# huettern/edison

Measured on AMD Instinct MI355X. Metric: MFCC frames/sec + KWS inferences/sec (whole node) at 1/2/4/8 MI355X, higher is better.
Workload: dtype f32

## Files before the change

### edison_amd/csrc/tables.c

```c
#include <math.h>
#include <stdio.h>
#include <stdlib.h>
#include <string.h>

#include "../../include/edison_hip.h"
#include "edison_internal.h"

#define MEL_HIGH_FREQUENCY_Q 1127.0
#define MEL_BREAK_FREQUENCY_HERTZ 700.0

static double hz2mel(double hz) { return MEL_HIGH_FREQUENCY_Q * log(1.0 + hz / MEL_BREAK_FREQUENCY_HERTZ); }

static void linspace(double a, double b, int n, double *out)
{
	double step = n > 1 ? (b - a) / (double)(n - 1) : 0.0;
	for (int i = 0; i < n; i++) out[i] = (double)i * step + a;
	if (n > 1) out[n - 1] = b;
}

int ed_gen_mel_weight_matrix(int num_mel_bins, int num_spectrogram_bins, double sample_rate,
                             double lower_edge_hertz, double upper_edge_hertz, double *W)
{
	if (num_mel_bins < 1 || num_spectrogram_bins < 2 || W == NULL) return EDISON_E_ARGUMENT;
	double *lin = (double *)malloc(sizeof(double) * (size_t)num_spectrogram_bins);
	double *edge = (double *)malloc(sizeof(double) * (size_t)(num_mel_bins + 2));
	if (!lin || !edge) { free(lin); free(edge); return EDISON_E_NO_MEMORY; }
	linspace(0.0, sample_rate / 2.0, num_spectrogram_bins, lin);
	linspace(hz2mel(lower_edge_hertz), hz2mel(upper_edge_hertz), num_mel_bins + 2, edge);
	memset(W, 0, sizeof(double) * (size_t)num_mel_bins);
	for (int k = 1; k < num_spectrogram_bins; k++)
	{
		double m = hz2mel(lin[k]);
		double *row = W + (size_t)k * num_mel_bins;
		for (int j = 0; j < num_mel_bins; j++)
		{
			double up = (m - edge[j]) / (edge[j + 1] - edge[j]);
			double dn = (edge[j + 2] - m) / (edge[j + 2] - edge[j + 1]);
			double w = up < dn ? up : dn;
			row[j] = w > 0.0 ? w : 0.0;
		}
	}
	free(lin); free(edge);
	return EDISON_OK;
}

static const unsigned char g_b128_group[4][16] = {
	{0, 1, 2, 3, 12, 13, 14, 15, 20, 21, 22, 23, 24, 25, 26, 27},
	{4, 5, 6, 7, 8, 9, 10, 11, 16, 17, 18, 19, 28, 29, 30, 31},
	{32, 33, 34, 35, 44, 45, 46, 47, 52, 53, 54, 55, 56, 57, 58, 59},
	{36, 37, 38, 39, 40, 41, 42, 43, 48, 49, 50, 51, 60, 61, 62, 63}};

static int mel_read_passes(int first4[2][EDISON_NUM_MEL][4], int NLO, int NHI, const int *col_band, const int *half)
{
	int total = 0;
	for (int part = 0; part < 2; part++)
		for (int t = 0; t < (part == 0 ? NLO : NHI); t++)
			for (int second = 0; second < 2; second++)
				for (int g = 0; g < 4; g++)
				{
					int n_in_slot[16] = {0}, held[16][16], worst = 1;
					for (int i = 0; i < 16; i++)
					{
						const int l = g_b128_group[g][i], b = col_band[l & 15];
						const int q = first4[part][part == 0 ? b : 31 - b][l >> 4] + t;
						const int addr = 2 * q + (second ? 1 - half[l] : half[l]), slot = addr & 15;
						int k = 0;
						while (k < n_in_slot[slot] && held[slot][k] != addr) k++;
						if (k == n_in_slot[slot]) held[slot][n_in_slot[slot]++] = addr;
						if (n_in_slot[slot] > worst) worst = n_in_slot[slot];
					}
					total += worst;
				}
	return total;
}

static void choose_lane_assignment(int first4[2][EDISON_NUM_MEL][4], int NLO, int NHI, int *col_band, int *half)
{
	int best = -1, cb[16], hf[64];
	uint32_t rng = 12345u;
	for (int start = 0; start < 8; start++)
	{
		for (int c = 0; c < 16; c++) cb[c] = c;
		for (int l = 0; l < 64; l++) hf[l] = l & 1;
		if (start > 0)
		{
			for (int c = 15; c > 0; c--)
			{
				rng = rng * 1664525u + 1013904223u;
				const int k = (int)((rng >> 8) % (uint32_t)(c + 1)), tmp = cb[c];
				cb[c] = cb[k]; cb[k] = tmp;
			}
			for (int l = 0; l < 64; l++) { rng = rng * 1664525u + 1013904223u; hf[l] = (int)((rng >> 16) & 1u); }
		}
		int cost = mel_read_passes(first4, NLO, NHI, cb, hf), improved = 1;
		while (improved)
		{
			improved = 0;
			for (int l = 0; l < 64; l++)
			{
				hf[l] ^= 1;
				const int c2 = mel_read_passes(first4, NLO, NHI, cb, hf);
				if (c2 < cost) { cost = c2; improved = 1; } else hf[l] ^= 1;
			}
			for (int a = 0; a < 16; a++)
				for (int b = a + 1; b < 16; b++)
				{
					int tmp = cb[a]; cb[a] = cb[b]; cb[b] = tmp;
					const int c2 = mel_read_passes(first4, NLO, NHI, cb, hf);
					if (c2 < cost) { cost = c2; improved = 1; } else { tmp = cb[a]; cb[a] = cb[b]; cb[b] = tmp; }
				}
		}
		if (best < 0 || cost < best)
		{
			best = cost;
			memcpy(col_band, cb, sizeof(cb));
			memcpy(half, hf, sizeof(hf));
		}
	}
}

int ed_build_mfcc_tables(int variant, double sample_rate, double lower_edge_hertz, double upper_edge_hertz,
                         double mel_mtx_scale, ed_mfcc_tables_t *out, char *err, size_t err_cap)
{
	const int NMEL = EDISON_NUM_MEL;
	const int nbins = (variant == EDISON_MFCC_A) ? EDISON_FRAME_LEN / 2 : EDISON_FRAME_LEN / 2 + 1;
	if (variant != EDISON_MFCC_A && variant != EDISON_MFCC_B && variant != EDISON_MFCC_TF) return EDISON_E_ARGUMENT;
	memset(out, 0, sizeof(*out));
	const double spec_scale = (variant == EDISON_MFCC_B) ? 0.5 / 1024.0 / sqrt(2.0) : 0.5;

	for (int l = 0; l < 64; l++)
		for (int p = 0; p < 8; p++)
		{
			double a = -2.0 * M_PI * (double)(l * p) / 512.0;
			out->tw1[p][l][0] = (float)cos(a); out->tw1[p][l][1] = (float)sin(a);
			a = -2.0 * M_PI * (double)((l & 7) * p) / 64.0;
			out->tw2[p][l][0] = (float)cos(a); out->tw2[p][l][1] = (float)sin(a);
		}
	for (int m = 0; m < 4; m++)
		for (int l = 0; l < 64; l++)
		{
			const int k0 = ED_K0(l);
			double a = -2.0 * M_PI * (double)(k0 + 64 * m) / 1024.0;
			out->twp[m][l][0] = (float)cos(a); out->twp[m][l][1] = (float)sin(a);
		}

	double *W = (double *)malloc(sizeof(double) * (size_t)nbins * NMEL);
	if (!W) return EDISON_E_NO_MEMORY;
	int r = ed_gen_mel_weight_matrix(NMEL, nbins, sample_rate, lower_edge_hertz, upper_edge_hertz, W);
	if (r != EDISON_OK) { free(W); return r; }
	(void)mel_mtx_scale;
	int q0[EDISON_NUM_MEL], nq[EDISON_NUM_MEL], ks[EDISON_NUM_MEL], ke[EDISON_NUM_MEL];
	for (int j = 0; j < NMEL; j++)
	{
		int first = -1, last = -1;
		for (int k = 0; k < nbins; k++)
			if (W[(size_t)k * NMEL + j] != 0.0) { if (first < 0) first = k; last = k; }
		if (first < 0) { first = 0; last = -1; }
		ks[j] = first; ke[j] = last + 1;
		q0[j] = first / 4;
		nq[j] = last >= first ? last / 4 - first / 4 + 1 : 0;
	}
	int NLO = 1, NHI = 1;
	for (int b = 0; b < 16; b++)
	{
		if ((nq[b] + 3) / 4 > NLO) NLO = (nq[b] + 3) / 4;
		if ((nq[31 - b] + 3) / 4 > NHI) NHI = (nq[31 - b] + 3) / 4;
	}
	if (NLO > ED_MEL_NLO_MAX || NHI > ED_MEL_NHI_MAX)
	{
		if (err) snprintf(err, err_cap, "mel filterbank needs %d+%d spectrum quads per lane, the kernel's budget is %d+%d",
		                  NLO, NHI, ED_MEL_NLO_MAX, ED_MEL_NHI_MAX);
		free(W);
		return EDISON_E_NO_IMPL;
	}
	const char *force_wide = getenv("EDISON_FORCE_WIDE_MEL");
	if (NLO <= 2 && NHI <= 5 && !(force_wide && force_wide[0] == '1')) { NLO = 2; NHI = 5; }
	else { NLO = ED_MEL_NLO_MAX; NHI = ED_MEL_NHI_MAX; }
	out->mel_NLO = NLO; out->mel_NHI = NHI;
	int first4[2][EDISON_NUM_MEL][4];
	for (int j = 0; j < NMEL; j++)
		for (int rr = 0; rr < 4; rr++)
			for (int part = 0; part < 2; part++)
			{
				const int N = part == 0 ? NLO : NHI;
				int s4 = q0[j] + rr * ((nq[j] + 3) / 4);
				if (s4 > ED_SPEC_QUADS - N) s4 = ED_SPEC_QUADS - N;
				if (s4 < 0) s4 = 0;
				first4[part][j][rr] = s4;
			}
	int col_band[16], half[64];
	choose_lane_assignment(first4, NLO, NHI, col_band, half);
	for (int l = 0; l < 64; l++)
	{
		const int b = col_band[l & 15], rr = l >> 4;
		out->mel_band[l] = b;
		out->mel_half[l] = half[l];
		for (int part = 0; part < 2; part++)
		{
			const int j = part == 0 ? b : 31 - b, N = part == 0 ? NLO : NHI;
			const int per = (nq[j] + 3) / 4;
			const int pq0 = q0[j] + rr * per;
			int pq1 = pq0 + per;
			if (pq1 > q0[j] + nq[j]) pq1 = q0[j] + nq[j];
			const int s4 = first4[part][j][rr];
			if (part == 0) out->mel_slo4[l] = s4; else out->mel_shi4[l] = s4;
			for (int t = 0; t < N; t++)
				for (int c = 0; c < 4; c++)
				{
					const int q = s4 + t, k = 4 * q + c;
					const int mine = q >= pq0 && q < pq1 && k >= ks[j] && k < ke[j] && k < nbins;
					out->mel_w4[(part == 0 ? 0 : NLO) + t][l][c] = mine ? (float)(spec_scale * W[(size_t)k * NMEL + j]) : 0.0f;
				}
		}
	}
	free(W);

	double dscale = (variant == EDISON_MFCC_B) ? 1.0 / 64.0 : 1.0 / sqrt(2.0 * (double)NMEL);
	for (int l = 0; l < 64; l++)
	{
		int c = l & 31, h = l >> 5;
		for (int n = 0; n < 8; n++)
		{
			int nn = n + 8 * h;
			out->dct4[n / 4][l][n % 4] =
			    (float)(dscale * 2.0 * cos(M_PI * (double)c * (double)(2 * nn + 1) / (double)(2 * NMEL)));
		}
	}
	out->spec_scale = (float)spec_scale;
	out->log_offset = 1e-6f;
	out->always_log = (variant == EDISON_MFCC_B) ? 0 : 1;
	if (variant == EDISON_MFCC_TF)
	{
		out->has_window = 1;
		for (int n = 0; n < EDISON_FRAME_LEN; n++)
			out->window2[n / 2][n % 2] = (float)(0.5 - 0.5 * cos(2.0 * M_PI * (double)n / (double)EDISON_FRAME_LEN));
	}
	return EDISON_OK;
}

enum { LDS_R128, LDS_W128, LDS_W64, LDS_W32, LDS_R2_64, LDS_RTN32 };

static void lds_passes(int kind, const int *addr, int *free_passes, int *extra_passes)
{
	const int n_groups = kind == LDS_R128 ? 4 : kind == LDS_W128 ? 8 : kind == LDS_W64 || kind == LDS_R2_64 ? 4 : 2;
	const int n_banks = kind == LDS_R128 ? 64 : 32;
	const int n_dwords = kind == LDS_R128 || kind == LDS_W128 ? 4 : kind == LDS_W64 || kind == LDS_R2_64 ? 2 : 1;
	const int per = 64 / n_groups;
	*free_passes = 0; *extra_passes = 0;
	for (int g = 0; g < n_groups; g++)
	{
		int n_in_bank[64] = {0}, held[64][32], worst = 0;
		for (int i = 0; i < per; i++)
		{
			const int l = kind == LDS_R128 ? g_b128_group[g][i] : g * per + i;
			if (addr[l] < 0) continue;
			for (int d = 0; d < n_dwords; d++)
			{
				const int dw = addr[l] / 4 + d, bank = dw % n_banks;
				int k = 0;
				while (k < n_in_bank[bank] && held[bank][k] != dw) k++;
				if (k == n_in_bank[bank]) held[bank][n_in_bank[bank]++] = dw;
				if (n_in_bank[bank] > worst) worst = n_in_bank[bank];
			}
		}
		if (worst > 0) { *free_passes += 1; *extra_passes += worst - 1; }
	}
}

int ed_mfcc2_lds_account(const ed_mfcc_tables_t *tab, int t2_stride, int wave, ed_lds_row_t *rows, int max_rows)
{
	if (!tab || !rows || max_rows < ED_LDS_ROWS_MAX || wave < 0 || t2_stride < 64) return EDISON_E_ARGUMENT;
	const int NLO = tab->mel_NLO, NHI = tab->mel_NHI;
	const int melw = 4 * ED2_TABLE_FLOATS;
	const int xbuf = 4 * (ED2_TABLE_FLOATS + (NLO + NHI) * 256 + wave * ED2_XBUF_FLOATS);
	const int S2 = xbuf + 4 * ED2_S_OFF, Lb2 = xbuf + 4 * ED2_L_OFF;
	int n = 0, addr[64], f, e;
#define ROW(nm, k) { rows[n].name = nm; rows[n].kind = k; rows[n].instructions = 0; rows[n].free_passes = 0; rows[n].extra_passes = 0; n++; }
#define ADD() { lds_passes(rows[n - 1].kind, addr, &f, &e); rows[n - 1].free_passes += f; rows[n - 1].extra_passes += e; }
#define ADD1() { ADD(); rows[n - 1].instructions++; }
	ROW("queue draw: ds_add_rtn_u32, lane 0", LDS_RTN32);
	for (int l = 0; l < 64; l++) addr[l] = l == 0 ? xbuf + 4 * (12 - wave) * ED2_XBUF_FLOATS : -1;
	ADD1();
	ROW("transpose 2 stores: ds_write_b128 xc4[stride (lane & 7) + (lane >> 3) + 8 q]", LDS_W128);
	for (int q = 0; q < 8; q++)
	{
		for (int l = 0; l < 64; l++) addr[l] = xbuf + 16 * (t2_stride * (l & 7) + (l >> 3) + 8 * q);
		ADD1();
	}
	ROW("transpose 2 reads: ds_read_b128 xc4[stride c + lane]", LDS_R128);
	for (int c = 0; c < 8; c++)
	{
		for (int l = 0; l < 64; l++) addr[l] = xbuf + 16 * (t2_stride * c + l);
		ADD1();
	}
	ROW("split twiddles: ds_read2st64_b64 tpl[64 m + lane], two m each", LDS_R2_64);
	for (int m = 0; m < 4; m++)
	{
		for (int l = 0; l < 64; l++) addr[l] = 4 * 512 + 8 * (64 * m + l);
		ADD();
		rows[n - 1].instructions = (m + 2) / 2;
	}
	ROW("spectrum stores: ds_write_b64 S2[k0 + 64 m]", LDS_W64);
	for (int m = 0; m < 4; m++)
	{
		for (int l = 0; l < 64; l++) addr[l] = S2 + 8 * (ED_K0(l) + 64 * m);
		ADD1();
	}
	ROW("spectrum stores, mirrored: ds_write_b64 S2[512 - k0 - 64 m]", LDS_W64);
	for (int m = 0; m < 4; m++)
	{
		for (int l = 0; l < 64; l++) addr[l] = S2 + 8 * (512 - ED_K0(l) - 64 * m);
		ADD1();
	}
	ROW("spectrum store S2[256]: ds_write_b64, lane 0", LDS_W64);
	for (int l = 0; l < 64; l++) addr[l] = l == 0 ? S2 + 8 * 256 : -1;
	ADD1();
	ROW("mel spectrum reads: ds_read_b128 S4[2 (first + t) + half], S4[2 (first + t) + 1 - half]", LDS_R128);
	for (int part = 0; part < 2; part++)
		for (int t = 0; t < (part == 0 ? NLO : NHI); t++)
			for (int second = 0; second < 2; second++)
			{
				for (int l = 0; l < 64; l++)
				{
					const int first = part == 0 ? tab->mel_slo4[l] : tab->mel_shi4[l], h = tab->mel_half[l];
					addr[l] = S2 + 16 * (2 * (first + t) + (second ? 1 - h : h));
					if (addr[l] + 16 > S2 + 8 * 516) return EDISON_E_ARGUMENT;
				}
				ADD1();
			}
	ROW("mel weight reads: ds_read_b128 melw4[64 t + lane]", LDS_R128);
	for (int t = 0; t < NLO + NHI; t++)
	{
		for (int l = 0; l < 64; l++) addr[l] = melw + 16 * (64 * t + l);
		ADD1();
	}
	ROW("DCT input store: ds_write_b32 Lb2[l_idx]", LDS_W32);
	for (int l = 0; l < 64; l++) addr[l] = Lb2 + 4 * (2 * (16 * ((l >> 4) & 1) + tab->mel_band[l]) + (l >> 5));
	ADD1();
	ROW("DCT input reads: ds_read_b128 L4[0..3], L4 = Lb2 + 16 (lane & 1) + 8 (lane >> 5)", LDS_R128);
	for (int i = 0; i < 4; i++)
	{
		for (int l = 0; l < 64; l++) addr[l] = Lb2 + 8 * (16 * (l & 1) + 8 * (l >> 5)) + 16 * i;
		ADD1();
	}
	ROW("DCT table reads: ds_read_b128 dctl[lane], dctl[64 + lane]", LDS_R128);
	for (int i = 0; i < 2; i++)
	{
		for (int l = 0; l < 64; l++) addr[l] = 16 * (64 * i + l);
		ADD1();
	}
#undef ROW
#undef ADD
#undef ADD1
	return n;
}

int ed_build_exact_tables(double sample_rate, double lower_edge_hertz, double upper_edge_hertz, double mel_mtx_scale, ed_exact_tables_t *out)
{
	const int NMEL = EDISON_NUM_MEL, nbins = EDISON_FRAME_LEN / 2 + 1;
	memset(out, 0, sizeof(*out));
	for (int k = 0; k < 512; k++)
	{
		out->tw[k][0] = cos(-2.0 * M_PI * (double)k / 1024.0);
		out->tw[k][1] = sin(-2.0 * M_PI * (double)k / 1024.0);
	}
	for (int c = 0; c < NMEL; c++)
		for (int n = 0; n < NMEL; n++)
			out->dct[c][n] = 2.0 * cos(M_PI * (double)c * (double)(2 * n + 1) / (double)(2 * NMEL));
	double *W = (double *)malloc(sizeof(double) * (size_t)nbins * NMEL);
	if (!W) return EDISON_E_NO_MEMORY;
	int r = ed_gen_mel_weight_matrix(NMEL, nbins, sample_rate, lower_edge_hertz, upper_edge_hertz, W);
	if (r != EDISON_OK) { free(W); return r; }
	int off = 0;
	for (int j = 0; j < NMEL; j++)
	{
		int first = -1, last = -1;
		for (int k = 0; k < nbins; k++)
			if (W[(size_t)k * NMEL + j] != 0.0) { if (first < 0) first = k; last = k; }
		const int len = first < 0 ? 0 : last - first + 1;
		if (off + len > ED_EXACT_TAPS_MAX) { free(W); return EDISON_E_NO_IMPL; }
		out->mel_off[j] = off; out->mel_k0[j] = first < 0 ? 0 : first; out->mel_len[j] = len;
		for (int t = 0; t < len; t++) out->mel_w[off + t] = mel_mtx_scale * W[(size_t)(first + t) * NMEL + j];
		off += len;
	}
	out->mel_div = mel_mtx_scale;
	free(W);
	return EDISON_OK;
}
```

Measured before the change: 1.507 billion.

## Search mel lane assignment with slack-aware start offsets to cut LDS bank conflicts

Adds a host-side randomized local search over the mel filterbank lane assignment. It varies band-to-column mapping, per-lane start quads within the range where the weights are nonzero, and the half-swap bit, scoring each candidate with an LDS bank-conflict model. The goal is fewer extra passes on the ds_read_b128 spectrum reads in the MFCC kernel. Table build time goes up, which a memo mitigates, and the model of bank behavior may not match the hardware.

Result: no change. 1.519 billion (median of 5 runs) (+0.8%).

```diff
diff --git a/edison_amd/csrc/tables.c b/edison_amd/csrc/tables.c
--- a/edison_amd/csrc/tables.c
+++ b/edison_amd/csrc/tables.c
@@ -1,4 +1,6 @@
+#include <limits.h>
 #include <math.h>
+#include <pthread.h>
 #include <stdio.h>
 #include <stdlib.h>
 #include <string.h>
@@ -44,11 +46,63 @@
 	return EDISON_OK;
 }
 
+enum { LDS_R128, LDS_W128, LDS_W64, LDS_W32, LDS_R2_64, LDS_RTN32 };
+
 static const unsigned char g_b128_group[4][16] = {
 	{0, 1, 2, 3, 12, 13, 14, 15, 20, 21, 22, 23, 24, 25, 26, 27},
 	{4, 5, 6, 7, 8, 9, 10, 11, 16, 17, 18, 19, 28, 29, 30, 31},
 	{32, 33, 34, 35, 44, 45, 46, 47, 52, 53, 54, 55, 56, 57, 58, 59},
 	{36, 37, 38, 39, 40, 41, 42, 43, 48, 49, 50, 51, 60, 61, 62, 63}};
+
+static int lds_groups(int kind) { return kind == LDS_R128 ? 4 : kind == LDS_W128 ? 8 : kind == LDS_W64 || kind == LDS_R2_64 ? 4 : 2; }
+
+static int lds_group_passes(int kind, int g, const int *addr, int *crowding)
+{
+	const int n_banks = kind == LDS_R128 ? 64 : 32;
+	const int n_dwords = kind == LDS_R128 || kind == LDS_W128 ? 4 : kind == LDS_W64 || kind == LDS_R2_64 ? 2 : 1;
+	const int per = 64 / lds_groups(kind);
+	int n_in_bank[64] = {0}, held[64][32], worst = 0, step = 1;
+	if (n_dwords == 4)
+	{
+		step = 4;
+		for (int i = 0; i < per; i++)
+		{
+			const int l = kind == LDS_R128 ? g_b128_group[g][i] : g * per + i;
+			if (addr[l] >= 0 && addr[l] % 16 != 0) step = 1;
+		}
+	}
+	for (int i = 0; i < per; i++)
+	{
+		const int l = kind == LDS_R128 ? g_b128_group[g][i] : g * per + i;
+		if (addr[l] < 0) continue;
+		for (int d = 0; d < n_dwords; d += step)
+		{
+			const int dw = addr[l] / 4 + d, bank = dw % n_banks;
+			int k = 0;
+			while (k < n_in_bank[bank] && held[bank][k] != dw) k++;
+			if (k == n_in_bank[bank]) held[bank][n_in_bank[bank]++] = dw;
+			if (n_in_bank[bank] > worst) worst = n_in_bank[bank];
+		}
+	}
+	if (crowding)
+	{
+		*crowding = 0;
+		for (int bank = 0; bank < n_banks; bank += step) *crowding += step * n_in_bank[bank] * n_in_bank[bank];
+	}
+	return worst;
+}
+
+static void lds_passes(int kind, const int *addr, int *free_passes, int *extra_passes)
+{
+	*free_passes = 0; *extra_passes = 0;
+	for (int g = 0; g < lds_groups(kind); g++)
+	{
+		const int worst = lds_group_passes(kind, g, addr, NULL);
+		if (worst > 0) { *free_passes += 1; *extra_passes += worst - 1; }
+	}
+}
+
+static int mel_read_slot(int first, int t, int second, int half) { return 2 * (first + t) + (second ? 1 - half : half); }
 
 static int mel_read_passes(int first4[2][EDISON_NUM_MEL][4], int NLO, int NHI, const int *col_band, const int *half)
 {
@@ -119,6 +173,144 @@
 	}
 }
 
+typedef struct
+{
+	int first_lo[2][16][4], first_hi[2][16][4], half_free[16][4];
+} mel_freedom_t;
+
+typedef struct
+{
+	int col_band[16], first[2][16][4], half[16][4];
+} mel_assignment_t;
+
+static long mel_group_cost(const mel_assignment_t *a, int part, int N, int g)
+{
+	long cost = 0;
+	int addr[64];
+	for (int t = 0; t < N; t++)
+		for (int second = 0; second < 2; second++)
+		{
+			int crowding;
+			for (int i = 0; i < 16; i++)
+			{
+				const int l = g_b128_group[g][i], b = a->col_band[l & 15], rr = l >> 4;
+				addr[l] = 16 * mel_read_slot(a->first[part][b][rr], t, second, a->half[b][rr]);
+			}
+			cost += (1L << 20) * lds_group_passes(LDS_R128, g, addr, &crowding) + crowding;
+		}
+	return cost;
+}
+
+static long mel_cost(const mel_assignment_t *a, int NLO, int NHI, long limit)
+{
+	long cost = 0;
+	for (int g = 0; g < 4 && cost < limit; g++)
+	{
+		cost += mel_group_cost(a, 0, NLO, g);
+		if (cost < limit) cost += mel_group_cost(a, 1, NHI, g);
+	}
+	return cost;
+}
+
+static void refine_lane_assignment(const mel_freedom_t *fr, int NLO, int NHI, mel_assignment_t *a)
+{
+	const int N[2] = {NLO, NHI};
+	int group_of[64];
+	for (int g = 0; g < 4; g++)
+		for (int i = 0; i < 16; i++) group_of[g_b128_group[g][i]] = g;
+	for (int round = 0, improved = 1; improved && round < 64; round++)
+	{
+		improved = 0;
+		for (int c = 0; c < 16; c++)
+			for (int rr = 0; rr < 4; rr++)
+			{
+				const int b = a->col_band[c], g = group_of[c + 16 * rr];
+				for (int part = 0; part < 2; part++)
+				{
+					int best_first = a->first[part][b][rr];
+					long best = mel_group_cost(a, part, N[part], g);
+					for (int s = fr->first_lo[part][b][rr]; s <= fr->first_hi[part][b][rr]; s++)
+					{
+						a->first[part][b][rr] = s;
+						const long c2 = mel_group_cost(a, part, N[part], g);
+						if (c2 < best) { best = c2; best_first = s; improved = 1; }
+					}
+					a->first[part][b][rr] = best_first;
+				}
+				if (fr->half_free[b][rr])
+				{
+					const long c1 = mel_group_cost(a, 0, NLO, g) + mel_group_cost(a, 1, NHI, g);
+					a->half[b][rr] ^= 1;
+					if (mel_group_cost(a, 0, NLO, g) + mel_group_cost(a, 1, NHI, g) < c1) improved = 1; else a->half[b][rr] ^= 1;
+				}
+			}
+		long cost = mel_cost(a, NLO, NHI, LONG_MAX);
+		for (int x = 0; x < 16; x++)
+			for (int y = x + 1; y < 16; y++)
+			{
+				if (group_of[x] == group_of[y]) continue;
+				int tmp = a->col_band[x]; a->col_band[x] = a->col_band[y]; a->col_band[y] = tmp;
+				const long c2 = mel_cost(a, NLO, NHI, cost);
+				if (c2 < cost) { cost = c2; improved = 1; } else { tmp = a->col_band[x]; a->col_band[x] = a->col_band[y]; a->col_band[y] = tmp; }
+			}
+	}
+}
+
+#ifndef ED_MEL_SEARCH_STARTS
+#define ED_MEL_SEARCH_STARTS 24
+#endif
+#define ED_MEL_SEARCH_MEMO 8
+static void search_lane_assignment(const mel_freedom_t *fr, int NLO, int NHI, mel_assignment_t *a)
+{
+	static struct { int used, NLO, NHI; mel_freedom_t fr; mel_assignment_t given, found; } memo[ED_MEL_SEARCH_MEMO];
+	static int memo_next = 0;
+	static pthread_mutex_t memo_lock = PTHREAD_MUTEX_INITIALIZER;
+	const mel_assignment_t given = *a;
+	pthread_mutex_lock(&memo_lock);
+	for (int i = 0; i < ED_MEL_SEARCH_MEMO; i++)
+		if (memo[i].used && memo[i].NLO == NLO && memo[i].NHI == NHI && !memcmp(&memo[i].fr, fr, sizeof(*fr)) && !memcmp(&memo[i].given, &given, sizeof(given)))
+		{
+			*a = memo[i].found;
+			pthread_mutex_unlock(&memo_lock);
+			return;
+		}
+	pthread_mutex_unlock(&memo_lock);
+	long best = -1;
+	uint32_t rng = 12345u;
+	for (int start = 0; start < ED_MEL_SEARCH_STARTS; start++)
+	{
+		mel_assignment_t c = given;
+		if (start > 0)
+		{
+			for (int x = 15; x > 0; x--)
+			{
+				rng = rng * 1664525u + 1013904223u;
+				const int k = (int)((rng >> 8) % (uint32_t)(x + 1)), tmp = c.col_band[x];
+				c.col_band[x] = c.col_band[k]; c.col_band[k] = tmp;
+			}
+			for (int b = 0; b < 16; b++)
+				for (int rr = 0; rr < 4; rr++)
+				{
+					for (int part = 0; part < 2; part++)
+					{
+						rng = rng * 1664525u + 1013904223u;
+						c.first[part][b][rr] = fr->first_lo[part][b][rr] + (int)((rng >> 8) % (uint32_t)(fr->first_hi[part][b][rr] - fr->first_lo[part][b][rr] + 1));
+					}
+					rng = rng * 1664525u + 1013904223u;
+					if (fr->half_free[b][rr] && ((rng >> 16) & 1u)) c.half[b][rr] ^= 1;
+				}
+		}
+		refine_lane_assignment(fr, NLO, NHI, &c);
+		const long cost = mel_cost(&c, NLO, NHI, LONG_MAX);
+		if (best < 0 || cost < best) { best = cost; *a = c; }
+	}
+	pthread_mutex_lock(&memo_lock);
+	memo[memo_next].used = 1; memo[memo_next].NLO = NLO; memo[memo_next].NHI = NHI;
+	memo[memo_next].fr = *fr; memo[memo_next].given = given; memo[memo_next].found = *a;
+	memo_next = (memo_next + 1) % ED_MEL_SEARCH_MEMO;
+	pthread_mutex_unlock(&memo_lock);
+}
+
 int ed_build_mfcc_tables(int variant, double sample_rate, double lower_edge_hertz, double upper_edge_hertz,
                          double mel_mtx_scale, ed_mfcc_tables_t *out, char *err, size_t err_cap)
 {
@@ -173,6 +365,7 @@
 		free(W);
 		return EDISON_E_NO_IMPL;
 	}
+	const int need_lo = NLO, need_hi = NHI;
 	const char *force_wide = getenv("EDISON_FORCE_WIDE_MEL");
 	if (NLO <= 2 && NHI <= 5 && !(force_wide && force_wide[0] == '1')) { NLO = 2; NHI = 5; }
 	else { NLO = ED_MEL_NLO_MAX; NHI = ED_MEL_NHI_MAX; }
@@ -190,11 +383,53 @@
 			}
 	int col_band[16], half[64];
 	choose_lane_assignment(first4, NLO, NHI, col_band, half);
+	mel_freedom_t fr;
+	mel_assignment_t as;
+	for (int c = 0; c < 16; c++)
+	{
+		const int b = col_band[c];
+		as.col_band[c] = b;
+		for (int rr = 0; rr < 4; rr++)
+		{
+			as.half[b][rr] = half[c + 16 * rr];
+			fr.half_free[b][rr] = 1;
+			for (int part = 0; part < 2; part++)
+			{
+				const int j = part == 0 ? b : 31 - b, N = part == 0 ? NLO : NHI;
+				const int n_used = part == 0 ? (need_lo > 2 ? N : 2) : (need_hi > 5 ? N : 5);
+				const int per = (nq[j] + 3) / 4, pq0 = q0[j] + rr * per;
+				int pq1 = pq0 + per, need0 = -1, need1 = -1;
+				if (pq1 > q0[j] + nq[j]) pq1 = q0[j] + nq[j];
+				for (int q = pq0; q < pq1; q++)
+				{
+					int nz[4];
+					for (int cc = 0; cc < 4; cc++)
+					{
+						const int k = 4 * q + cc;
+						nz[cc] = k >= ks[j] && k < ke[j] && k < nbins && (float)(spec_scale * W[(size_t)k * NMEL + j]) != 0.0f;
+					}
+					if (nz[0] || nz[1] || nz[2] || nz[3]) { if (need0 < 0) need0 = q; need1 = q + 1; }
+					if ((nz[0] && nz[2]) || (nz[1] && nz[3])) fr.half_free[b][rr] = 0;
+				}
+				int lo = 0, hi = ED_SPEC_QUADS - N;
+				if (need0 >= 0)
+				{
+					if (need1 - n_used > lo) lo = need1 - n_used;
+					if (need0 < hi) hi = need0;
+				}
+				const int s4 = first4[part][j][rr];
+				if (s4 < lo || s4 > hi) lo = hi = s4;
+				as.first[part][b][rr] = s4;
+				fr.first_lo[part][b][rr] = lo; fr.first_hi[part][b][rr] = hi;
+			}
+		}
+	}
+	search_lane_assignment(&fr, NLO, NHI, &as);
 	for (int l = 0; l < 64; l++)
 	{
-		const int b = col_band[l & 15], rr = l >> 4;
+		const int b = as.col_band[l & 15], rr = l >> 4;
 		out->mel_band[l] = b;
-		out->mel_half[l] = half[l];
+		out->mel_half[l] = as.half[b][rr];
 		for (int part = 0; part < 2; part++)
 		{
 			const int j = part == 0 ? b : 31 - b, N = part == 0 ? NLO : NHI;
@@ -202,7 +437,7 @@
 			const int pq0 = q0[j] + rr * per;
 			int pq1 = pq0 + per;
 			if (pq1 > q0[j] + nq[j]) pq1 = q0[j] + nq[j];
-			const int s4 = first4[part][j][rr];
+			const int s4 = as.first[part][b][rr];
 			if (part == 0) out->mel_slo4[l] = s4; else out->mel_shi4[l] = s4;
 			for (int t = 0; t < N; t++)
 				for (int c = 0; c < 4; c++)
@@ -236,35 +471,6 @@
 			out->window2[n / 2][n % 2] = (float)(0.5 - 0.5 * cos(2.0 * M_PI * (double)n / (double)EDISON_FRAME_LEN));
 	}
 	return EDISON_OK;
-}
-
-enum { LDS_R128, LDS_W128, LDS_W64, LDS_W32, LDS_R2_64, LDS_RTN32 };
-
-static void lds_passes(int kind, const int *addr, int *free_passes, int *extra_passes)
-{
-	const int n_groups = kind == LDS_R128 ? 4 : kind == LDS_W128 ? 8 : kind == LDS_W64 || kind == LDS_R2_64 ? 4 : 2;
-	const int n_banks = kind == LDS_R128 ? 64 : 32;
-	const int n_dwords = kind == LDS_R128 || kind == LDS_W128 ? 4 : kind == LDS_W64 || kind == LDS_R2_64 ? 2 : 1;
-	const int per = 64 / n_groups;
-	*free_passes = 0; *extra_passes = 0;
-	for (int g = 0; g < n_groups; g++)
-	{
-		int n_in_bank[64] = {0}, held[64][32], worst = 0;
-		for (int i = 0; i < per; i++)
-		{
-			const int l = kind == LDS_R128 ? g_b128_group[g][i] : g * per + i;
-			if (addr[l] < 0) continue;
-			for (int d = 0; d < n_dwords; d++)
-			{
-				const int dw = addr[l] / 4 + d, bank = dw % n_banks;
-				int k = 0;
-				while (k < n_in_bank[bank] && held[bank][k] != dw) k++;
-				if (k == n_in_bank[bank]) held[bank][n_in_bank[bank]++] = dw;
-				if (n_in_bank[bank] > worst) worst = n_in_bank[bank];
-			}
-		}
-		if (worst > 0) { *free_passes += 1; *extra_passes += worst - 1; }
-	}
 }
 
 int ed_mfcc2_lds_account(const ed_mfcc_tables_t *tab, int t2_stride, int wave, ed_lds_row_t *rows, int max_rows)
@@ -323,7 +529,7 @@
 				for (int l = 0; l < 64; l++)
 				{
 					const int first = part == 0 ? tab->mel_slo4[l] : tab->mel_shi4[l], h = tab->mel_half[l];
-					addr[l] = S2 + 16 * (2 * (first + t) + (second ? 1 - h : h));
+					addr[l] = S2 + 16 * mel_read_slot(first, t, second, h);
 					if (addr[l] + 16 > S2 + 8 * 516) return EDISON_E_ARGUMENT;
 				}
 				ADD1();
```
